# heyoeyo/muggled_dpt

Hardware: AMD Instinct MI355X
Metric: depth-maps/sec @518x518 (504x504 model tensor), Depth-Anything-V2 ViT-L (higher is better)
Workload: dtype bf16; 1 GPU; Depth-Anything-V2 ViT-L (vitl), 518x518 image -> 504x504 tensor, batch 32/GPU, bf16 MFMA operands + fp32 accumulate, mdpt_forward via C ABI; global_batch=32, parallelism=dp1, gemm_tile=0, batch_split=True

## Files before the change

### muggled_dpt_amd/csrc/gemm.hip

```cpp

#include "mdpt_kernels.h"
#include "mdpt_prof.h"
#include "f8_cross.h"
#include <stdio.h>
#include <stdlib.h>

#pragma clang fp contract(off)

typedef __attribute__((ext_vector_type(16))) float f32x16;
typedef __attribute__((ext_vector_type(4))) float f32x4;

namespace {

#include "gemm_common.inc"
#include "gemm_epilogue_strip.inc"
#include "gemm_lockstep.inc"
#include "gemm8_epilogues.inc"
#include "gemm8.inc"

template <int AMODE, int EKIND, int DMODE, bool F8 = false>
int launch_pp_mode(const GemmParams& p, hipStream_t stream) {
    constexpr unsigned LDS = 2 * 65536;
    if constexpr (MDPT_OP_IS_F16 && !F8 && (EKIND == MDPT_E_GENERIC || EKIND == MDPT_E_D2S) && DMODE != DM_RINIT) {
        if (p.f8) return launch_pp_mode<AMODE, EKIND, DMODE, true>(p, stream);
    }
    auto kern = gemm8_kernel<AMODE, EKIND, DMODE, F8>;
    static bool attr_done = false;
    if (!attr_done) {
        hipError_t e = hipFuncSetAttribute((const void*)kern, hipFuncAttributeMaxDynamicSharedMemorySize, LDS);
        if (e != hipSuccess) return (int)e;
        attr_done = true;
    }
    const int tiles = ((p.M + 255) / 256) * ((p.N + 255) / 256);
    static char prof_name[64] = "";
    if (!prof_name[0]) snprintf(prof_name, sizeof(prof_name), F8 ? "gemm8_kernel<%d, %d, %d, f8>" : "gemm8_kernel<%d, %d, %d>", AMODE, EKIND, DMODE);
    MdptProfScope prof(prof_name, 2.0 * (p.M_alg > 0 ? p.M_alg : p.M) * p.N * p.K, stream);
    const int ks = (AMODE == MDPT_A_DENSE && EKIND == MDPT_E_GENERIC && DMODE == DM_F32 && p.ksplit > 1) ? p.ksplit : 1;
    hipLaunchKernelGGL(kern, dim3(tiles, ks), dim3(512), LDS, stream, p);
    return (int)hipGetLastError();
}

template <int AMODE, int EKIND>
int launch_pp(const GemmParams& p, hipStream_t stream) {
    if constexpr (EKIND == MDPT_E_GENERIC) {
        const int dmode = generic_direct_mode(p);
// ... 134 lines not shown
```

### muggled_dpt_amd/csrc/gemm8.inc

```
template <int AMODE, bool F8 = false>
struct HalfStager {
    static constexpr int A_BYTES = 256 * 128;
#ifdef MDPT_GEMM8_BUF_STAGING
    static constexpr bool BUFFERED = AMODE != MDPT_A_CONV3;
#else
    static constexpr bool BUFFERED = false;
#endif
    __amdgpu_buffer_rsrc_t rs_a, rs_w;
    unsigned a_voff[4], b_voff;
    int a_soff, b_soff, a_row_step, b_row_step;
    const op_t* a_base_hi; const op_t* a_base_lo; const op_t* w_base_hi; const op_t* w_base_lo;
    size_t a_bytes, w_bytes;
    const op_t* a_ptr[4];
    int a_pix[4], a_y[4], a_x[4], a_ko[4];
    const op_t* b_ptr[4];
    ptrdiff_t a_hi_minus_lo, w_lo_minus_hi;
    const op_t* conv_plane;
    int a_pass, a_k0, a_tap, a_ci, b_pass, b_k0;
    int st_m0, st_n0, b_step;
    bool a_f8, b_f8;

    __device__ __forceinline__ void place_a(const GemmParams& p, int pass, int wave, int lane) {
        const int lrow = lane >> 3;
        a_f8 = pass < p.npass - 1;
// ... 188 lines not shown
        }
        }
        if (F8 && H == 1 && b_f8) {
            b_k0 += 128;
            if (b_k0 == p.K) {
                b_k0 = 0;
                ++b_pass;
                place_b(p, b_pass, wave, threadIdx.x & 63);
            }
        } else
        if (H == 1) {
            b_k0 += 64;
            if (b_k0 == p.K) {
                b_k0 = 0;
                const ptrdiff_t dw = (b_pass == 0 ? w_lo_minus_hi : -w_lo_minus_hi) - p.K;
#pragma unroll
                for (int i = 0; i < 4; ++i) b_ptr[i] += dw;
                ++b_pass;
            }
        }
    }
};

template <int AMODE, int EKIND, bool SW, bool RI = false, bool FAST = false, bool F8 = false>
__device__ __forceinline__ void gemm8_body(const GemmParams& p, char* smem, const int dmode, const int m0, const int n0,
                                           const unsigned long long t_start) {
    static_assert(!RI || SW, "residual-initialised accumulators use the swapped operand order (4 consecutive columns per lane)");
    static_assert(!F8 || (!FAST && !RI && MDPT_HAVE_F8), "fp8 cross terms: state-machine stager, fp16 build");
    static_assert(!FAST || AMODE == MDPT_A_DENSE, "the stateless staging is for dense rows");
    constexpr int A_BYTES = 256 * 128, BUF = 2 * A_BYTES;
    const int tid = threadIdx.x, lane = tid & 63;
    const int wave = __builtin_amdgcn_readfirstlane(tid >> 6);
    const int grp = wave >> 2, wc = wave & 3;
    unsigned long long t_first = 0, t_loop = 0;
    constexpr bool swapped = SW;
    HalfStager<AMODE, F8> st;
    if constexpr (!FAST) st.init(p, m0, n0, wave, lane);
    typedef __attribute__((address_space(3))) void* lds_ptr_t;
    __amdgpu_buffer_rsrc_t rs_a, rs_w;
    unsigned fa_voff = 0, fb_voff = 0;
    int fa_step = 0, fb_step = 0;
    if constexpr (FAST) {
        const int rows_here = p.M - m0 < 256 ? p.M - m0 : 256, cols_here = p.N - n0 < 256 ? p.N - n0 : 256;
        rs_a = tile_rsrc(p.A_hi + (size_t)m0 * p.lda, (size_t)rows_here * p.lda * 2);
        rs_w = tile_rsrc(p.W_hi + (size_t)n0 * p.ldw, ((size_t)(cols_here - 1) * p.ldw + p.K) * 2);
        const int r = wave * 8 + (lane >> 3);
        const int koff = ((lane & 7) ^ ((r >> 1) & 7)) * 8;
        fa_voff = (unsigned)(r * p.lda + koff) * 2u;
        fb_voff = (unsigned)(r * p.ldw + koff) * 2u;
        fa_step = 64 * p.lda * 2;
        fb_step = 64 * p.ldw * 2;
    }
#define ISSUE_A(H_, BUF_, KB_)                                                                                          \
    do {                                                                                                                \
        if constexpr (FAST) {                                                                                           \
            _Pragma("unroll") for (int i = 2 * (H_); i < 2 * (H_) + 2; ++i)                                             \
                __builtin_amdgcn_raw_ptr_buffer_load_lds(rs_a, (lds_ptr_t)((BUF_) + (wave + 8 * i) * 1024), 16, fa_voff, (KB_) + i * fa_step, 0, 0); \
        } else {                                                                                                        \
            st.template issue_a<H_>(p, BUF_, wave);                                                                     \
        }                                                                                                               \
    } while (0)
#define ISSUE_B(H_, BUF_, KB_)                                                                                          \
    do {                                                                                                                \
        if constexpr (FAST) {                                                                                           \
            _Pragma("unroll") for (int i = 2 * (H_); i < 2 * (H_) + 2; ++i)                                             \
                __builtin_amdgcn_raw_ptr_buffer_load_lds(rs_w, (lds_ptr_t)((BUF_) + 256 * 128 + (wave + 8 * i) * 1024), 16, fb_voff, (KB_) + i * fb_step, 0, 0); \
        } else {                                                                                                        \
            st.template issue_b<H_>(p, BUF_, wave);                                                                     \
        }                                                                                                               \
    } while (0)

    const int l15 = lane & 15, lh = lane >> 4, key = (l15 >> 1) & 7;
    const int a_off0 = (grp * 64 + l15) * 128 + ((lh ^ key) << 4), a_off1 = (grp * 64 + l15) * 128 + (((4 + lh) ^ key) << 4);
    const int b_off0 = A_BYTES + (wc * 32 + l15) * 128 + ((lh ^ key) << 4), b_off1 = A_BYTES + (wc * 32 + l15) * 128 + (((4 + lh) ^ key) << 4);

// ... 52 lines not shown
    do {                                                                                                              \
        if constexpr (swapped) f8_mfma16_w_first<2 * (QN_) + (J_)>(acc[QM_][QN_][I_][J_], f8_cat(FB_[J_][0], FB_[J_][1]), f8_cat(fa[I_][0], fa[I_][1]), WS_, asc); \
        else f8_mfma16_a_first<2 * (QN_) + (J_)>(acc[QM_][QN_][I_][J_], f8_cat(fa[I_][0], fa[I_][1]), f8_cat(FB_[J_][0], FB_[J_][1]), asc, WS_); \
    } while (0)
#define MFMA_Q8(QM_, QN_, FB_, WS_)                                                                                   \
    do {                                                                                                              \
        __builtin_amdgcn_s_setprio(1);                                                                                \
        MFMA_Q8_ONE(QM_, QN_, FB_, 0, 0, WS_); MFMA_Q8_ONE(QM_, QN_, FB_, 0, 1, WS_);                                 \
        MFMA_Q8_ONE(QM_, QN_, FB_, 1, 0, WS_); MFMA_Q8_ONE(QM_, QN_, FB_, 1, 1, WS_);                                 \
        MFMA_Q8_ONE(QM_, QN_, FB_, 2, 0, WS_); MFMA_Q8_ONE(QM_, QN_, FB_, 2, 1, WS_);                                 \
        MFMA_Q8_ONE(QM_, QN_, FB_, 3, 0, WS_); MFMA_Q8_ONE(QM_, QN_, FB_, 3, 1, WS_);                                 \
        __builtin_amdgcn_s_setprio(0);                                                                                \
    } while (0)
#endif
#define WAIT_LGKM(N_) asm volatile("s_waitcnt lgkmcnt(" #N_ ")" ::: "memory")
#define WAIT_VM(N_) asm volatile("s_waitcnt vmcnt(" #N_ ")" ::: "memory")
#define ACC_READY(QM_, QN_, N_)                                                                                                          \
    asm volatile("s_waitcnt vmcnt(" #N_ ")"                                                                                              \
                 : "+v"(acc[QM_][QN_][0][0]), "+v"(acc[QM_][QN_][0][1]), "+v"(acc[QM_][QN_][1][0]), "+v"(acc[QM_][QN_][1][1]),           \
                   "+v"(acc[QM_][QN_][2][0]), "+v"(acc[QM_][QN_][2][1]), "+v"(acc[QM_][QN_][3][0]), "+v"(acc[QM_][QN_][3][1])            \
                 :                                                                                                                       \
                 : "memory")

    const int T = F8 ? ktiles_total(p, p.K) : (p.K / 64) * p.npass;
    const int T8 = F8 ? ktiles_f8(p, p.K) : 0, T8a = F8 ? p.K / 128 : 0;
    char* const bufE = smem;
    char* const bufO = smem + BUF;
    ISSUE_A(0, bufE, 0);
    ISSUE_B(0, bufE, 0);
    ISSUE_B(1, bufE, 0);
    ISSUE_A(1, bufE, 0);
    if constexpr (RI) {
        constexpr unsigned OOB = 0xFFFFFFF0u;
        typedef __attribute__((ext_vector_type(4))) int i32x4;
        const int rows_here = p.M - m0 < 256 ? p.M - m0 : 256;
        const unsigned long long base = (unsigned long long)(p.resid + (size_t)m0 * p.ldr);
        i32x4 rs;
        rs[0] = __builtin_amdgcn_readfirstlane((int)(unsigned)base);
        rs[1] = __builtin_amdgcn_readfirstlane((int)(unsigned)(base >> 32) & 0xFFFF);
        rs[2] = __builtin_amdgcn_readfirstlane((int)(unsigned)((size_t)rows_here * p.ldr * 4));
        rs[3] = 0x00020000;
        const unsigned row_b = (unsigned)p.ldr * 4u;
        auto load_quadrant = [&](int qm, int qn) {
#pragma unroll
            for (int j = 0; j < 2; ++j) {
                const int nc = n0 + qn * 128 + wc * 32 + j * 16 + 4 * lh;
                const unsigned col = nc < p.N ? (unsigned)nc * 4u : OOB;
#pragma unroll
                for (int i = 0; i < 4; ++i) {
                    const unsigned row = (unsigned)(qm * 128 + grp * 64 + i * 16 + l15) * row_b;
                    const unsigned off = col == OOB ? OOB : row + col;
                    asm volatile("s_nop 4\n\tbuffer_load_dwordx4 %0, %1, %2, 0 offen" : "=v"(acc[qm][qn][i][j]) : "v"(off), "s"(rs) : "memory");
                }
            }
        };
        load_quadrant(0, 0);
        ISSUE_B(0, bufO, 128);
        ISSUE_A(0, bufO, 128);
        ISSUE_B(1, bufO, 128);
        ISSUE_A(1, bufO, 128);
        load_quadrant(0, 1);
        load_quadrant(1, 1);
        load_quadrant(1, 0);
        WAIT_VM(40);
    } else {
        ISSUE_B(0, bufO, 128);
        ISSUE_A(0, bufO, 128);
        ISSUE_B(1, bufO, 128);
        ISSUE_A(1, bufO, 128);
        WAIT_VM(8);
    }
    BAR();
    if (p.dbg_times) t_first = memtime_now();
    if (grp == 1) BAR();


    const float ri_scale = (MDPT_OP_IS_F16 && RI && p.wscale) ? p.wscale[0] : 1.0f;
#define SCALE_Q(QM_, QN_)                                                                                             \
    do {                                                                                                              \
        if (MDPT_OP_IS_F16 && RI && ri_scale != 1.0f) {                                                               \
            _Pragma("unroll") for (int i = 0; i < 4; ++i)                                                             \
                _Pragma("unroll") for (int j = 0; j < 2; ++j) acc[QM_][QN_][i][j] *= ri_scale;                        \
        }                                                                                                             \
    } while (0)
#define GEMM8_ITER(MORE_, FIRST_, MQ)                                                                                       \
    do {                                                                                                              \
        const int kE = t * 128 + 256, kO = kE + 128;         \
                                                                                                              \
        LOAD_B(fb0, 0, 0); PIN(); LOAD_A(0, 0); PIN();                                                                \
        WAIT_LGKM(8); BAR(); WAIT_LGKM(0); PIN();                                                                     \
        if (FIRST_) { ACC_READY(0, 0, 32); SCALE_Q(0, 0); PIN(); }                     \
        MQ(0, 0, fb0); BAR();                                                                                     \
                                                                                                              \
        LOAD_B(fb1, 1, 0); PIN();                                                                                     \
        if (MORE_) ISSUE_B(0, bufE, kE);                                                             \
        BAR(); WAIT_LGKM(0); PIN();                                                                                   \
        if (FIRST_) { ACC_READY(0, 1, 18); SCALE_Q(0, 1); PIN(); }                               \
        MQ(0, 1, fb1); BAR();                                                                                     \
                                                                                                              \
        LOAD_A(1, 0); PIN();                                                                                          \
        if (MORE_) ISSUE_A(0, bufE, kE);                                                             \
        PIN(); WAIT_LGKM(0); BAR(); PIN();                                                                            \
        if (FIRST_) { ACC_READY(1, 1, 12); SCALE_Q(1, 1); PIN(); }                                \
        MQ(1, 1, fb1); BAR();                                                                                     \
                                                                                                              \
        if (MORE_) { ISSUE_B(1, bufE, kE); ISSUE_A(1, bufE, kE); PIN(); WAIT_VM(8); } else { WAIT_VM(0); }                      \
        BAR();                                                                                                        \
        if (FIRST_) { ACC_READY(1, 0, 8); SCALE_Q(1, 0); PIN(); }  \
        MQ(1, 0, fb0); BAR();                                                                                     \
                                                                                                              \
        LOAD_B(fb0, 0, 1); PIN(); LOAD_A(0, 1); PIN();                                                                \
        WAIT_LGKM(8); BAR(); WAIT_LGKM(0); PIN();                                                                     \
        MQ(0, 0, fb0); BAR();                                                                                     \
                                                                                                              \
        LOAD_B(fb1, 1, 1); PIN();                                                                                     \
        if (MORE_) ISSUE_B(0, bufO, kO);                                                             \
        BAR(); WAIT_LGKM(0); PIN();                                                                                   \
        MQ(0, 1, fb1); BAR();                                                                                     \
                                                                                                              \
        LOAD_A(1, 1); PIN();                                                                                          \
        if (MORE_) ISSUE_A(0, bufO, kO);                                                             \
        PIN(); WAIT_LGKM(0); BAR(); PIN();                                                                            \
        MQ(1, 1, fb1); BAR();                                                                                     \
                                                                                                              \
        if (MORE_) { ISSUE_B(1, bufO, kO); ISSUE_A(1, bufO, kO); PIN(); WAIT_VM(8); }                                          \
        BAR();                                                                                                        \
        MQ(1, 0, fb0); BAR();                                                                                     \
    } while (0)
    if constexpr (FAST) {
        int t = 0;
        if constexpr (RI) {
            GEMM8_ITER(true, true, MFMA_Q);
            t = 2;
        }
        for (; t + 2 < T; t += 2) GEMM8_ITER(true, false, MFMA_Q);
        GEMM8_ITER(false, false, MFMA_Q);
    } else {
        int t = 0;
#if MDPT_HAVE_F8
        if constexpr (F8) {
#define MQ8A(QM_, QN_, FB_) MFMA_Q8(QM_, QN_, FB_, wsc)
#define MQ8B(QM_, QN_, FB_) MFMA_Q8(QM_, QN_, FB_, wsc_lo)
            for (; t < T8a; t += 2) GEMM8_ITER(true, false, MQ8A);
            for (; t < T8; t += 2) GEMM8_ITER(true, false, MQ8B);
#undef MQ8A
#undef MQ8B
        }
#endif
        for (; t < T; t += 2) {
            const bool more = t + 2 < T;
            GEMM8_ITER(more, (RI && t == 0), MFMA_Q);
        }
    }
#undef GEMM8_ITER
#undef SCALE_Q
#undef ACC_READY
#undef ISSUE_A
#undef ISSUE_B
    if (grp == 0) BAR();
#undef LOAD_A
#undef LOAD_B
#undef MFMA_Q
#if MDPT_HAVE_F8
#undef MFMA_Q8
#undef MFMA_Q8_ONE
#endif
    if (p.dbg_times) t_loop = memtime_now();
    if constexpr (SW) {
        if (EKIND == MDPT_E_SWQKV) {
            if (dmode == DM_F32) {
                if (HAVE_IMGB && p.bias_img_stride) epilogue_direct<DM_F32, false, MDPT_ACT_NONE, HAVE_IMGB>(p, acc, m0, n0, grp, wc, lane);
                else epilogue_direct<DM_F32, false, MDPT_ACT_NONE>(p, acc, m0, n0, grp, wc, lane);
            } else if (HAVE_IMGB && p.bias_img_stride) {
                if (p.q_lo) epilogue_swin_qk<true, HAVE_IMGB>(p, acc, m0, n0, grp, wc, lane);
// ... 16 lines not shown
            } else {
                if (p.out_lo) epilogue_direct<DM_BF16, true, MDPT_ACT_NONE, HAVE_IMGB>(p, acc, m0, n0, grp, wc, lane);
                else epilogue_direct<DM_BF16, false, MDPT_ACT_NONE, HAVE_IMGB>(p, acc, m0, n0, grp, wc, lane);
            }
        } else if (dmode == DM_BF16) {
            const int sel = (p.out_lo ? 3 : 0) + (p.act == MDPT_ACT_GELU ? 2 : (p.act == MDPT_ACT_RELU || p.relu_bf16) ? 1 : 0);
            switch (sel) {
                case 0: epilogue_direct<DM_BF16, false, MDPT_ACT_NONE>(p, acc, m0, n0, grp, wc, lane); break;
                case 1: epilogue_direct<DM_BF16, false, MDPT_ACT_RELU>(p, acc, m0, n0, grp, wc, lane); break;
                case 2: epilogue_direct<DM_BF16, false, MDPT_ACT_GELU>(p, acc, m0, n0, grp, wc, lane); break;
                case 3: epilogue_direct<DM_BF16, true, MDPT_ACT_NONE>(p, acc, m0, n0, grp, wc, lane); break;
                case 4: epilogue_direct<DM_BF16, true, MDPT_ACT_RELU>(p, acc, m0, n0, grp, wc, lane); break;
                default: epilogue_direct<DM_BF16, true, MDPT_ACT_GELU>(p, acc, m0, n0, grp, wc, lane); break;
            }
        } else if (dmode == DM_F32 || dmode == DM_RINIT) {
            if (HAVE_IMGB && p.bias_img_stride) epilogue_direct<DM_F32, false, MDPT_ACT_NONE, HAVE_IMGB>(p, acc, m0, n0, grp, wc, lane);
            else epilogue_direct<DM_F32, false, MDPT_ACT_NONE>(p, acc, m0, n0, grp, wc, lane);
        } else {
            epilogue_direct<DM_RESID, false, MDPT_ACT_NONE>(p, acc, m0, n0, grp, wc, lane);
        }
        if (p.dbg_times && tid == 0) {
            const unsigned long long t_issued = memtime_now();
            asm volatile("s_waitcnt vmcnt(0)" ::: "memory");
            unsigned long long* d = p.dbg_times + (size_t)blockIdx.x * 6;
            d[0] = t_start; d[1] = t_first; d[2] = t_loop; d[3] = memtime_now();
            d[4] = t_issued;
            d[5] = __builtin_amdgcn_s_getreg(4 << 0 | 0 << 6 | 31 << 11);
        }
        return;
    }
    if ((EKIND == MDPT_E_QKV && dmode == DM_VT) || (EKIND == MDPT_E_SWQKV && dmode == DM_SWVT)) {
        if (EKIND == MDPT_E_SWQKV) {
            if (HAVE_IMGB && p.bias_img_stride) {
                if (p.vt_lo) epilogue_swin_vt<true, HAVE_IMGB>(p, acc, m0, n0, grp, wc, lane);
                else epilogue_swin_vt<false, HAVE_IMGB>(p, acc, m0, n0, grp, wc, lane);
            } else if (p.vt_lo) epilogue_swin_vt<true>(p, acc, m0, n0, grp, wc, lane);
            else epilogue_swin_vt<false>(p, acc, m0, n0, grp, wc, lane);
        } else if (HAVE_IMGB && p.bias_img_stride) {
            if (p.vt_lo) epilogue_direct_vt<true, HAVE_IMGB>(p, acc, m0, n0, grp, wc, lane);
            else epilogue_direct_vt<false, HAVE_IMGB>(p, acc, m0, n0, grp, wc, lane);
        } else if (p.vt_lo) {
            epilogue_direct_vt<true>(p, acc, m0, n0, grp, wc, lane);
        } else {
            epilogue_direct_vt<false>(p, acc, m0, n0, grp, wc, lane);
        }
        if (p.dbg_times && tid == 0) {
            asm volatile("s_waitcnt vmcnt(0)" ::: "memory");
// ... 23 lines not shown
        asm volatile("s_waitcnt vmcnt(0)" ::: "memory");
        unsigned long long* d = p.dbg_times + (size_t)blockIdx.x * 6;
        d[0] = t_start; d[1] = t_first; d[2] = t_loop; d[3] = memtime_now();
        d[4] = __builtin_amdgcn_s_getreg(20 << 0 | 0 << 6 | 3 << 11);
        d[5] = __builtin_amdgcn_s_getreg(4 << 0 | 0 << 6 | 31 << 11);
    }
}
#undef PIN
#undef BAR
#undef WAIT_LGKM
#undef WAIT_VM

__host__ __device__ inline int generic_direct_mode(const GemmParams& p) {
    const bool imgb_ok = HAVE_IMGB && p.bias_img_rows >= 256 && p.bias && !p.gamma && !p.relu_bf16 && p.act != MDPT_ACT_RELU;
    const bool plain = !p.up_src && (!p.bias_img_stride || imgb_ok);
    const bool fits = (size_t)256 * p.ldc * 4 < 0xFFFFFFF0ull;
    if (plain && fits && p.out_hi && !p.out_f32 && !p.gamma && !p.resid && !(p.relu_bf16 && p.act != MDPT_ACT_NONE)) return DM_BF16;
    if (plain && fits && !p.bias_img_stride && p.out_f32 && !p.out_hi && p.gamma && p.resid && p.resid == p.out_f32 && p.bias && p.act == MDPT_ACT_NONE && p.ldr == p.ldc)
        return DM_RESID;
    if (plain && fits && p.acc_init && p.out_f32 && !p.out_hi && !p.gamma && p.resid == p.out_f32 && p.ldr == p.ldc && p.act == MDPT_ACT_NONE && !p.relu_bf16)
        return DM_RINIT;
    if (plain && fits && p.out_f32 && !p.out_hi && !p.gamma && !p.resid && p.act == MDPT_ACT_NONE && !p.relu_bf16) return DM_F32;
    return DM_NONE;
}

template <int AMODE, int EKIND, int DMODE, bool F8 = false>
__global__ __launch_bounds__(512, 1) void gemm8_kernel(const GemmParams p) {
    extern __shared__ __attribute__((aligned(16))) char smem[];
    unsigned long long t_start = 0;
    if (p.dbg_times) t_start = memtime_now();
    int m0, n0;
    tile_coords((p.N + 255) / 256, 256, 256, m0, n0);
    if constexpr (EKIND == MDPT_E_SWQKV) {
        const bool fast = p.npass == 1;
        if (n0 >= 2 * p.F && p.swin_vtokmap) {
            if (fast) gemm8_body<AMODE, EKIND, false, false, true>(p, smem, DM_SWVT, m0, n0, t_start);
            else gemm8_body<AMODE, EKIND, false>(p, smem, DM_SWVT, m0, n0, t_start);
        } else {
            const int dm = n0 >= 2 * p.F ? DM_F32 : DM_SWQK;
            if (fast) gemm8_body<AMODE, EKIND, true, false, true>(p, smem, dm, m0, n0, t_start);
            else gemm8_body<AMODE, EKIND, true>(p, smem, dm, m0, n0, t_start);
        }
    } else if (EKIND == MDPT_E_QKV) {
#ifdef MDPT_GEMM8_NO_FAST
        const bool fast = false;
#else
// ... 49 lines not shown
```

### muggled_dpt_amd/csrc/gemm8_epilogues.inc

```
constexpr bool HAVE_IMGB = MDPT_OP_IS_F16 != 0;
enum { DM_NONE = 0, DM_BF16 = 1, DM_RESID = 2, DM_QK = 3, DM_VT = 4, DM_F32 = 5, DM_RINIT = 6, DM_SWQK = 7, DM_SWVT = 8 };

__device__ __forceinline__ __amdgpu_buffer_rsrc_t tile_rsrc(const void* base, size_t bytes) {
    return __builtin_amdgcn_make_buffer_rsrc(const_cast<void*>(base), 0, (int)(unsigned)(bytes < 0xFFFFFFF0ull ? bytes : 0xFFFFFFF0ull), 0x00020000);
}

template <int MODE, bool X3, int ACT, bool IMGB = false>
__device__ __forceinline__ void epilogue_direct(const GemmParams& p, f32x4 (&acc)[2][2][4][2], int m0, int n0, int grp, int wc, int lane) {
    typedef __attribute__((ext_vector_type(2))) float f32x2;
    typedef __attribute__((ext_vector_type(4))) unsigned u32x4;
    constexpr unsigned OOB = 0xFFFFFFF0u;
    const int l15 = lane & 15, lh = lane >> 4;
    const int rows_here = p.M - m0 < 256 ? p.M - m0 : 256;
    int bnd = 1 << 30;
    const float* bias0 = p.bias;
    const float* bias1 = p.bias;
    if (IMGB) {
        const int img0 = m0 / p.bias_img_rows;
        bnd = (img0 + 1) * p.bias_img_rows - m0;
        bias0 = p.bias + (size_t)img0 * p.bias_img_stride;
        bias1 = bnd < rows_here ? bias0 + p.bias_img_stride : bias0;
    }
    auto pick = [&](const f32x4& a, const f32x4& b, bool next) {
        f32x4 r;
#pragma unroll
        for (int e = 0; e < 4; ++e) r[e] = next ? b[e] : a[e];
        return r;
    };

    if (MODE == DM_F32) {
        const __amdgpu_buffer_rsrc_t rs = tile_rsrc(p.out_f32 + (size_t)m0 * p.ldc, (size_t)rows_here * p.ldc * 4);
        const unsigned row_b = (unsigned)p.ldc * 4u;
        const float inv_s = (MDPT_OP_IS_F16 && p.wscale) ? p.wscale[1] : 1.0f;
#pragma unroll
        for (int qn = 0; qn < 2; ++qn) {
            f32x4 bias[2], biasn[2];
            unsigned col_off[2];
#pragma unroll
            for (int j = 0; j < 2; ++j) {
                const int nc = n0 + qn * 128 + wc * 32 + j * 16 + 4 * lh;
                bias[j] = p.bias ? *(const f32x4*)(bias0 + (nc < p.N ? nc : p.N - 4)) : f32x4{0.0f, 0.0f, 0.0f, 0.0f};
                if (IMGB) biasn[j] = *(const f32x4*)(bias1 + (nc < p.N ? nc : p.N - 4));
                col_off[j] = nc < p.N ? (unsigned)nc * 4u : OOB;
            }
#pragma unroll
            for (int qm = 0; qm < 2; ++qm)
#pragma unroll
                for (int i = 0; i < 4; ++i) {
                    const unsigned row = (unsigned)(qm * 128 + grp * 64 + i * 16 + l15) * row_b;
                    const bool next = IMGB && qm * 128 + grp * 64 + i * 16 + l15 >= bnd;
#pragma unroll
                    for (int j = 0; j < 2; ++j) {
                        const f32x4 a = MDPT_OP_IS_F16 ? acc[qm][qn][i][j] * inv_s : acc[qm][qn][i][j];
                        const f32x4 v = a + (IMGB ? pick(bias[j], biasn[j], next) : bias[j]);
                        __builtin_amdgcn_raw_buffer_store_b128(__builtin_bit_cast(u32x4, v), rs, col_off[j] == OOB ? OOB : row + col_off[j], 0, 0);
                    }
                }
        }
        return;
    }
    if (MODE == DM_RESID) {
        const __amdgpu_buffer_rsrc_t rs = tile_rsrc(p.out_f32 + (size_t)m0 * p.ldc, (size_t)rows_here * p.ldc * 4);
        const unsigned row_b = (unsigned)p.ldc * 4u;
        f32x4 bias[2][2], gam[2][2];
        unsigned col_off[2][2];
#pragma unroll
        for (int qn = 0; qn < 2; ++qn)
#pragma unroll
            for (int j = 0; j < 2; ++j) {
                const int nc = n0 + qn * 128 + wc * 32 + j * 16 + 4 * lh;
                const int ncl = nc < p.N ? nc : p.N - 4;
                bias[qn][j] = *(const f32x4*)(p.bias + ncl);
                gam[qn][j] = *(const f32x4*)(p.gamma + ncl);
                col_off[qn][j] = nc < p.N ? (unsigned)nc * 4u : OOB;
            }
        auto row_off = [&](int g, int i) { return (unsigned)((g >> 1) * 128 + grp * 64 + i * 16 + l15) * row_b; };
        u32x4 old[4][4][2];
        f32x4 res[2][4][2];
        auto load_group = [&](int g) {
#pragma unroll
// ... 454 lines not shown
```

### muggled_dpt_amd/csrc/gemm_common.inc

```
__device__ __forceinline__ void glds16(const void* gsrc, char* lds_wave_base) {
    __builtin_amdgcn_global_load_lds((const __attribute__((address_space(1))) void*)gsrc,
                                     (__attribute__((address_space(3))) void*)lds_wave_base, 16, 0, 0);
}

__device__ __forceinline__ unsigned long long memtime_now() {
    unsigned long long t;
    asm volatile("s_memtime %0\n\ts_waitcnt lgkmcnt(0)" : "=s"(t)::"memory");
    return t;
}

#define MDPT_GELU_Q0 1.1511051654815674f
#define MDPT_GELU_Q1 0.4592081904411316f
#define MDPT_GELU_Q2 0.052496179938316345f
#define MDPT_GELU_Q3 -0.00706342002376914f
#define MDPT_GELU_Q4 0.00013693643268197775f
#define MDPT_GELU_Q5 0.00018618021567817777f
#define MDPT_GELU_Q6 -3.93776863347739e-05f
#define MDPT_GELU_Q7 2.8349124931992264e-06f
__device__ __forceinline__ float gelu_erf(float v) {
    const float a = fabsf(v);
    float q = MDPT_GELU_Q7;
    q = __builtin_fmaf(q, a, MDPT_GELU_Q6);
    q = __builtin_fmaf(q, a, MDPT_GELU_Q5);
    q = __builtin_fmaf(q, a, MDPT_GELU_Q4);
// ... 172 lines not shown
        st_k0 += BK;
        if (AMODE == MDPT_A_CONV3) {
            st_sub += BK;
            if (st_sub == 64) {
                st_sub = 0;
                if (++st_tap == 9) { st_tap = 0; st_ci += 64; }
            }
        }
        if (st_k0 == kspan) {
            st_k0 = 0; st_tap = st_tap0; st_ci = st_ci0; st_sub = 0;
            const ptrdiff_t da = (st_pass == 0 ? a_hi_minus_lo : 0) - kspan;
            const ptrdiff_t dw = (st_pass == 0 ? w_lo_minus_hi : -w_lo_minus_hi) - kspan;
            if (st_pass == 0) conv_plane = p.A_hi;
#pragma unroll
            for (int i = 0; i < CA; ++i)
                if (AMODE != MDPT_A_CONV3) a_ptr[i] += da;
#pragma unroll
            for (int i = 0; i < CB; ++i) b_ptr[i] += dw;
            ++st_pass;
        }
    }
};

__device__ __forceinline__ void tile_coords(int tiles_n, int BM, int BN, int& m0, int& n0) {
    const int nwg = gridDim.x, bid = blockIdx.x;
    const int xq = nwg >> 3, xr = nwg & 7, xcd = bid & 7;
    const int swz = (xcd < xr ? xcd * (xq + 1) : xr * (xq + 1) + (xcd - xr) * xq) + (bid >> 3);
    if (tiles_n >= 8 && (tiles_n & 3) == 0) {
        const int tiles_m = nwg / tiles_n, per_panel = tiles_m * 4;
        const int panel = swz / per_panel, r = swz - panel * per_panel;
        m0 = (r >> 2) * BM;
        n0 = (panel * 4 + (r & 3)) * BN;
        return;
    }
    m0 = (swz / tiles_n) * BM;
    n0 = (swz % tiles_n) * BN;
}
```

### muggled_dpt_amd/csrc/mdpt_debug.cpp

```cpp
#include "mdpt_internal.h"

extern "C" {

int mdpt_debug_set_stop(mdpt_handle* h, int32_t block, int32_t step) {
    if (!h) return fail(MDPT_E_INVALID, "null handle");
    h->dbg_block = block; h->dbg_step = step;
    return 0;
}

int mdpt_debug_set_reassemble_overlap(mdpt_handle* h, int32_t on) {
    if (!h) return fail(MDPT_E_INVALID, "null handle");
    if (on < 0 || on > 2) return fail(MDPT_E_INVALID, "reassemble overlap: 0 = off, 1 = the library's rule, 2 = always");
    h->overlap_reasm = on;
    return 0;
}

int mdpt_debug_set_wscale_policy(mdpt_handle* h, int32_t all) {
    if (!h) return fail(MDPT_E_INVALID, "null handle");
    h->wscale_all = all ? 1 : 0;
    h->finalized = false;
    return 0;
}

int mdpt_debug_set_side_stream_priority(mdpt_handle* h, int32_t prio) {
// ... 85 lines not shown
    return 0;
}

int mdpt_debug_gemm(const void* a_bf16, const void* w_bf16, void* out_f32, void* out_bf16, int32_t M, int32_t N, int32_t K,
                    int32_t tile, int32_t iters, void* stream, void* dbg_times) {
    if (!a_bf16 || !w_bf16 || (!out_f32 && !out_bf16)) return fail(MDPT_E_INVALID, "null argument");
    GemmParams g;
    memset(&g, 0, sizeof(g));
    g.A_hi = (const op_t*)a_bf16; g.W_hi = (const op_t*)w_bf16;
    g.M = M; g.N = N; g.K = K; g.lda = K; g.npass = 1;
    g.zero_page = (const op_t*)w_bf16;
    g.amode = MDPT_A_DENSE; g.ekind = MDPT_E_GENERIC; g.tile = tile & 255;
    g.act = (tile >> 8) & 3;
    g.out_f32 = (float*)out_f32; g.out_hi = (op_t*)out_bf16; g.ldc = N; g.ldr = N;
    g.dbg_times = (unsigned long long*)dbg_times;
    if ((tile >> 10) & 1) {
        if (!out_f32 || !out_bf16) return fail(MDPT_E_INVALID, "residual mode needs both output buffers");
        g.bias = (const float*)out_bf16; g.gamma = (const float*)out_bf16 + N; g.resid = (const float*)out_f32; g.out_hi = nullptr;
    }
    if ((tile >> 11) & 1) {
        if (!out_f32 || !out_bf16) return fail(MDPT_E_INVALID, "residual mode needs both output buffers");
        g.bias = (const float*)out_bf16; g.resid = (const float*)out_f32; g.out_hi = nullptr; g.acc_init = 1;
    }
    for (int i = 0; i < iters; ++i) CHK(OPLG(mdpt_launch_gemm, g, (hipStream_t)stream));
    return 0;
}

int mdpt_debug_conv3(const void* in_bf16, const void* w_packed_bf16, const void* bias_f32, const void* skip_f32, const void* up_f32, int32_t Hu,
                     int32_t Wu, void* out_f32, void* out_bf16, int32_t relu_bf16, int32_t B, int32_t H, int32_t W, int32_t Cin, int32_t Cout,
                     int32_t path, int32_t tile, int32_t iters, void* stream, void* dbg_times, const void* in_lo_bf16, const void* w_lo_bf16,
                     void* out_lo_bf16) {
    if (Cout != 256 && Cout != 128) return fail(MDPT_E_INVALID, "Cout must be 256 or 128");
    if (w_lo_bf16 && !in_lo_bf16) return fail(MDPT_E_INVALID, "a lo plane of the weights needs one of the input (three passes); the input alone = two passes");
    if (!in_bf16 || !w_packed_bf16 || (!out_bf16 && !out_f32)) return fail(MDPT_E_INVALID, "null argument");
    static op_t* zero_page = nullptr;
    if (!zero_page) {
        if (hipMalloc((void**)&zero_page, 256) != hipSuccess || hipMemset(zero_page, 0, 256) != hipSuccess) return fail(MDPT_E_STATE, "zero page allocation failed");
    }
    if (path == 2 || path == 3) {
        if (Cout != 128 || !out_bf16 || Hu < 2 || Wu < 2) return fail(MDPT_E_INVALID, "upsampled-input form: 128 output channels, bf16 output");
        if (path == 2) {
            Conv3hParams q;
            memset(&q, 0, sizeof(q));
            q.up_in = (const op_t*)in_bf16; q.Hs = Hu; q.Ws = Wu; q.w = (const op_t*)w_packed_bf16; q.bias = (const float*)bias_f32;
            q.out_bf = (op_t*)out_bf16; q.B = B; q.H = H; q.W = W; q.Cin = Cin; q.Cout = 128;
            q.dbg_times = (unsigned long long*)dbg_times;
// ... 75 lines not shown
```

### muggled_dpt_amd/csrc/mdpt_kernels.h

```cpp
#pragma once
#include <hip/hip_runtime.h>
#include <stddef.h>
#include <stdint.h>

#include "op_types.h"

enum { MDPT_DT_F32 = 0, MDPT_DT_BF16 = 1, MDPT_DT_F16 = 2 };

enum { MDPT_A_DENSE = 0, MDPT_A_TOKENS = 1, MDPT_A_CONV3 = 2 };
enum { MDPT_E_GENERIC = 0, MDPT_E_QKV = 1, MDPT_E_PATCH = 2, MDPT_E_D2S = 3, MDPT_E_HEAD = 4, MDPT_E_SWQKV = 5 };
enum { MDPT_ACT_NONE = 0, MDPT_ACT_RELU = 1, MDPT_ACT_GELU = 2 };
enum { MDPT_TILE_AUTO = 0, MDPT_TILE_128x128 = 1, MDPT_TILE_256x256 = 2, MDPT_TILE_128x32 = 3, MDPT_TILE_256x128 = 4, MDPT_TILE_PP256 = 5, MDPT_TILE_64x64 = 6 };

struct GemmParams {
    const op_t* A_hi; const op_t* A_lo;
    const op_t* W_hi; const op_t* W_lo;
    int M, N, K;
    int ldw;
    int M_alg;
    int lda;
    int npass;
    const op_t* zero_page;
    int amode, ekind, tile;
    int tok_np, tok_stride;
// ... 1 lines not shown
    const float* bias; const float* gamma; const float* resid; int ldr;
    int bias_img_stride, bias_img_rows;
    const float* up_src; int Hu, Wu;
    int act;
    float* out_f32; op_t* out_hi; op_t* out_lo; int ldc;
    int relu_bf16;
    int acc_init;
    const float* wscale;
    op_t* q_hi; op_t* q_lo; op_t* k_hi; op_t* k_lo; op_t* vt_hi; op_t* vt_lo;
    int F, heads, npad, npadv; float qscale;
    const int* swin_tokmap; const float* swin_logit_scale; int swin_N, swin_img_rows;
    const int* swin_vtokmap; int swin_img_velems;
    const float* pos;
    int d2s_k, d2s_cout;
    const float* head_w; const float* head_b; int head_sigmoid; void* head_out; int head_out_dtype;
    int throughput_mode;
    int f8; size_t a8_off;
    const unsigned char* W8; const unsigned char* W8_lo;
    const unsigned char* S8; const unsigned char* S8_lo;
    size_t out_f8; int out_a8;
    int ksplit; float* ks_part;
    int ks_all;
    unsigned long long* dbg_times;
};


struct Conv3hParams {
    const op_t* in;
    const op_t* up_in; int Hs, Ws;
    const op_t* in_lo;
    const op_t* w;
    const op_t* w_lo;
    const float* bias;
    const float* skip;
    const float* up_src; int Hu, Wu;
    float* out_f32;
    op_t* out_bf;
    op_t* out_bf_lo;
    int relu_bf;
    int B, H, W, Cin;
    int Cout;
    int f8; size_t a8_off;
    const unsigned char* w8; const unsigned char* w8_lo; const unsigned char* s8; const unsigned char* s8_lo;
    size_t out_f8; int out_a8;
    unsigned long long* dbg_times;
};
// ... 114 lines not shown
```

Baseline: 768.8 depth-maps/s.

## Add persistent tile-walking kernel for residual-initialised dense GEMM

Adds a persistent variant of the residual-initialised (DM_RINIT) dense GEMM. One workgroup per CU loops over output tiles. It prefetches the next tile's operands while finishing the current one, and overlaps the previous tile's fp32 epilogue stores with the residual loads that initialise the next tile's accumulators. The aim is to hide per-tile prologue and epilogue latency and to remove wave-quantisation tails when tiles outnumber CUs. The cost is more complex control flow, register pressure, and new ACC_READY wait counts that must match the changed load ordering.

```diff
diff --git a/muggled_dpt_amd/csrc/gemm.hip b/muggled_dpt_amd/csrc/gemm.hip
--- a/muggled_dpt_amd/csrc/gemm.hip
+++ b/muggled_dpt_amd/csrc/gemm.hip
@@ -18,9 +18,44 @@
 #include "gemm8_epilogues.inc"
 #include "gemm8.inc"
 
+int rinit_persistent_grid(const GemmParams& p, int tiles) {
+    if (p.npass != 1 || (p.N & 255) || p.bias_img_stride || p.wscale || p.rinit_grid < 0) return 0;
+    if (p.rinit_grid > 0) return p.rinit_grid < tiles ? p.rinit_grid : tiles;
+#ifdef MDPT_DEBUG_SWITCHES
+    static const bool off = getenv("MDPT_GEMM_NO_PERSIST") != nullptr;
+    if (off) return 0;
+#endif
+    static int cus = 0;
+    if (!cus) {
+        int dev = 0, n = 0;
+        if (hipGetDevice(&dev) != hipSuccess || hipDeviceGetAttribute(&n, hipDeviceAttributeMultiprocessorCount, dev) != hipSuccess || n < 8) return 0;
+        cus = n & ~7;
+    }
+    return tiles >= 2 * cus ? cus : 0;
+}
+
+int launch_rinit_persistent(const GemmParams& p_in, int grid, hipStream_t stream) {
+    constexpr unsigned LDS = 2 * 65536;
+    static bool attr_done = false;
+    if (!attr_done) {
+        hipError_t e = hipFuncSetAttribute((const void*)gemm8_rinit_persistent_kernel, hipFuncAttributeMaxDynamicSharedMemorySize, LDS);
+        if (e != hipSuccess) return (int)e;
+        attr_done = true;
+    }
+    GemmParams p = p_in;
+    p.ptiles = ((p.M + 255) / 256) * ((p.N + 255) / 256);
+    MdptProfScope prof("gemm8_kernel<0, 0, 6, persistent>", 2.0 * (p.M_alg > 0 ? p.M_alg : p.M) * p.N * p.K, stream);
+    hipLaunchKernelGGL(gemm8_rinit_persistent_kernel, dim3(grid), dim3(512), LDS, stream, p);
+    return (int)hipGetLastError();
+}
+
 template <int AMODE, int EKIND, int DMODE, bool F8 = false>
 int launch_pp_mode(const GemmParams& p, hipStream_t stream) {
     constexpr unsigned LDS = 2 * 65536;
+    if constexpr (AMODE == MDPT_A_DENSE && EKIND == MDPT_E_GENERIC && DMODE == DM_RINIT && !F8) {
+        const int grid = rinit_persistent_grid(p, ((p.M + 255) / 256) * ((p.N + 255) / 256));
+        if (grid > 0) return launch_rinit_persistent(p, grid, stream);
+    }
     if constexpr (MDPT_OP_IS_F16 && !F8 && (EKIND == MDPT_E_GENERIC || EKIND == MDPT_E_D2S) && DMODE != DM_RINIT) {
         if (p.f8) return launch_pp_mode<AMODE, EKIND, DMODE, true>(p, stream);
     }
diff --git a/muggled_dpt_amd/csrc/gemm8.inc b/muggled_dpt_amd/csrc/gemm8.inc
--- a/muggled_dpt_amd/csrc/gemm8.inc
+++ b/muggled_dpt_amd/csrc/gemm8.inc
@@ -234,10 +234,11 @@
     }
 };
 
-template <int AMODE, int EKIND, bool SW, bool RI = false, bool FAST = false, bool F8 = false>
-__device__ __forceinline__ void gemm8_body(const GemmParams& p, char* smem, const int dmode, const int m0, const int n0,
-                                           const unsigned long long t_start) {
+template <int AMODE, int EKIND, bool SW, bool RI = false, bool FAST = false, bool F8 = false, bool PERSIST = false>
+__device__ __forceinline__ void gemm8_body(const GemmParams& p, char* smem, const int dmode, int m0, int n0,
+                                           unsigned long long t_start) {
     static_assert(!RI || SW, "residual-initialised accumulators use the swapped operand order (4 consecutive columns per lane)");
+    static_assert(!PERSIST || (RI && FAST), "the tile walk exists for the residual-initialised form with stateless staging");
     static_assert(!F8 || (!FAST && !RI && MDPT_HAVE_F8), "fp8 cross terms: state-machine stager, fp16 build");
     static_assert(!FAST || AMODE == MDPT_A_DENSE, "the stateless staging is for dense rows");
     constexpr int A_BYTES = 256 * 128, BUF = 2 * A_BYTES;
@@ -245,6 +246,7 @@
     const int wave = __builtin_amdgcn_readfirstlane(tid >> 6);
     const int grp = wave >> 2, wc = wave & 3;
     unsigned long long t_first = 0, t_loop = 0;
+    int vb = (int)blockIdx.x;
     constexpr bool swapped = SW;
     HalfStager<AMODE, F8> st;
     if constexpr (!FAST) st.init(p, m0, n0, wave, lane);
@@ -263,6 +265,11 @@
         fa_step = 64 * p.lda * 2;
         fb_step = 64 * p.ldw * 2;
     }
+    auto place_operands = [&](int tm0, int tn0) {
+        const int rows_here = p.M - tm0 < 256 ? p.M - tm0 : 256, cols_here = p.N - tn0 < 256 ? p.N - tn0 : 256;
+        rs_a = tile_rsrc(p.A_hi + (size_t)tm0 * p.lda, (size_t)rows_here * p.lda * 2);
+        rs_w = tile_rsrc(p.W_hi + (size_t)tn0 * p.ldw, ((size_t)(cols_here - 1) * p.ldw + p.K) * 2);
+    };
 #define ISSUE_A(H_, BUF_, KB_)                                                                                          \
     do {                                                                                                                \
         if constexpr (FAST) {                                                                                           \
@@ -361,6 +368,32 @@
                  :                                                                                                                       \
                  : "memory")
 
+    typedef __attribute__((ext_vector_type(4))) int i32x4;
+    i32x4 rs_r = {0, 0, 0, 0};
+    int r_n0 = n0;
+    auto resid_rsrc = [&](int tm0) {
+        const int rows_here = p.M - tm0 < 256 ? p.M - tm0 : 256;
+        const unsigned long long base = (unsigned long long)(p.resid + (size_t)tm0 * p.ldr);
+        rs_r[0] = __builtin_amdgcn_readfirstlane((int)(unsigned)base);
+        rs_r[1] = __builtin_amdgcn_readfirstlane((int)(unsigned)(base >> 32) & 0xFFFF);
+        rs_r[2] = __builtin_amdgcn_readfirstlane((int)(unsigned)((size_t)rows_here * p.ldr * 4));
+        rs_r[3] = 0x00020000;
+    };
+    auto load_quadrant = [&](int qm, int qn, int l15, int lh) {
+        constexpr unsigned OOB = 0xFFFFFFF0u;
+        const unsigned row_b = (unsigned)p.ldr * 4u;
+#pragma unroll
+        for (int j = 0; j < 2; ++j) {
+            const int nc = r_n0 + qn * 128 + wc * 32 + j * 16 + 4 * lh;
+            const unsigned col = nc < p.N ? (unsigned)nc * 4u : OOB;
+#pragma unroll
+            for (int i = 0; i < 4; ++i) {
+                const unsigned row = (unsigned)(qm * 128 + grp * 64 + i * 16 + l15) * row_b;
+                const unsigned off = col == OOB ? OOB : row + col;
+                asm volatile("s_nop 4\n\tbuffer_load_dwordx4 %0, %1, %2, 0 offen" : "=v"(acc[qm][qn][i][j]) : "v"(off), "s"(rs_r) : "memory");
+            }
+        }
+    };
     const int T = F8 ? ktiles_total(p, p.K) : (p.K / 64) * p.npass;
     const int T8 = F8 ? ktiles_f8(p, p.K) : 0, T8a = F8 ? p.K / 128 : 0;
     char* const bufE = smem;
@@ -369,38 +402,23 @@
     ISSUE_B(0, bufE, 0);
     ISSUE_B(1, bufE, 0);
     ISSUE_A(1, bufE, 0);
-    if constexpr (RI) {
-        constexpr unsigned OOB = 0xFFFFFFF0u;
-        typedef __attribute__((ext_vector_type(4))) int i32x4;
-        const int rows_here = p.M - m0 < 256 ? p.M - m0 : 256;
-        const unsigned long long base = (unsigned long long)(p.resid + (size_t)m0 * p.ldr);
-        i32x4 rs;
-        rs[0] = __builtin_amdgcn_readfirstlane((int)(unsigned)base);
-        rs[1] = __builtin_amdgcn_readfirstlane((int)(unsigned)(base >> 32) & 0xFFFF);
-        rs[2] = __builtin_amdgcn_readfirstlane((int)(unsigned)((size_t)rows_here * p.ldr * 4));
-        rs[3] = 0x00020000;
-        const unsigned row_b = (unsigned)p.ldr * 4u;
-        auto load_quadrant = [&](int qm, int qn) {
-#pragma unroll
-            for (int j = 0; j < 2; ++j) {
-                const int nc = n0 + qn * 128 + wc * 32 + j * 16 + 4 * lh;
-                const unsigned col = nc < p.N ? (unsigned)nc * 4u : OOB;
-#pragma unroll
-                for (int i = 0; i < 4; ++i) {
-                    const unsigned row = (unsigned)(qm * 128 + grp * 64 + i * 16 + l15) * row_b;
-                    const unsigned off = col == OOB ? OOB : row + col;
-                    asm volatile("s_nop 4\n\tbuffer_load_dwordx4 %0, %1, %2, 0 offen" : "=v"(acc[qm][qn][i][j]) : "v"(off), "s"(rs) : "memory");
-                }
-            }
-        };
-        load_quadrant(0, 0);
+    if constexpr (PERSIST) {
         ISSUE_B(0, bufO, 128);
         ISSUE_A(0, bufO, 128);
         ISSUE_B(1, bufO, 128);
         ISSUE_A(1, bufO, 128);
-        load_quadrant(0, 1);
-        load_quadrant(1, 1);
-        load_quadrant(1, 0);
+    } else
+    if constexpr (RI) {
+        resid_rsrc(m0);
+        r_n0 = n0;
+        load_quadrant(0, 0, l15, lh);
+        ISSUE_B(0, bufO, 128);
+        ISSUE_A(0, bufO, 128);
+        ISSUE_B(1, bufO, 128);
+        ISSUE_A(1, bufO, 128);
+        load_quadrant(0, 1, l15, lh);
+        load_quadrant(1, 1, l15, lh);
+        load_quadrant(1, 0, l15, lh);
         WAIT_VM(40);
     } else {
         ISSUE_B(0, bufO, 128);
@@ -409,10 +427,11 @@
         ISSUE_A(1, bufO, 128);
         WAIT_VM(8);
     }
-    BAR();
-    if (p.dbg_times) t_first = memtime_now();
-    if (grp == 1) BAR();
-
+    if constexpr (!PERSIST) {
+        BAR();
+        if (p.dbg_times) t_first = memtime_now();
+        if (grp == 1) BAR();
+    }
 
     const float ri_scale = (MDPT_OP_IS_F16 && RI && p.wscale) ? p.wscale[0] : 1.0f;
 #define SCALE_Q(QM_, QN_)                                                                                             \
@@ -422,25 +441,25 @@
                 _Pragma("unroll") for (int j = 0; j < 2; ++j) acc[QM_][QN_][i][j] *= ri_scale;                        \
         }                                                                                                             \
     } while (0)
-#define GEMM8_ITER(MORE_, FIRST_, MQ)                                                                                       \
+#define GEMM8_ITER(MORE_, FIRST_, MQ, R1_, R2_, R3_)                                                                                     \
     do {                                                                                                              \
         const int kE = t * 128 + 256, kO = kE + 128;         \
                                                                                                               \
         LOAD_B(fb0, 0, 0); PIN(); LOAD_A(0, 0); PIN();                                                                \
         WAIT_LGKM(8); BAR(); WAIT_LGKM(0); PIN();                                                                     \
-        if (FIRST_) { ACC_READY(0, 0, 32); SCALE_Q(0, 0); PIN(); }                     \
+        if (FIRST_) { ACC_READY(0, 0, R1_); SCALE_Q(0, 0); PIN(); }                  \
         MQ(0, 0, fb0); BAR();                                                                                     \
                                                                                                               \
         LOAD_B(fb1, 1, 0); PIN();                                                                                     \
         if (MORE_) ISSUE_B(0, bufE, kE);                                                             \
         BAR(); WAIT_LGKM(0); PIN();                                                                                   \
-        if (FIRST_) { ACC_READY(0, 1, 18); SCALE_Q(0, 1); PIN(); }                               \
+        if (FIRST_) { ACC_READY(0, 1, R2_); SCALE_Q(0, 1); PIN(); }                             \
         MQ(0, 1, fb1); BAR();                                                                                     \
                                                                                                               \
         LOAD_A(1, 0); PIN();                                                                                          \
         if (MORE_) ISSUE_A(0, bufE, kE);                                                             \
         PIN(); WAIT_LGKM(0); BAR(); PIN();                                                                            \
-        if (FIRST_) { ACC_READY(1, 1, 12); SCALE_Q(1, 1); PIN(); }                                \
+        if (FIRST_) { ACC_READY(1, 1, R3_); SCALE_Q(1, 1); PIN(); }                             \
         MQ(1, 1, fb1); BAR();                                                                                     \
                                                                                                               \
         if (MORE_) { ISSUE_B(1, bufE, kE); ISSUE_A(1, bufE, kE); PIN(); WAIT_VM(8); } else { WAIT_VM(0); }                      \
@@ -468,27 +487,85 @@
     } while (0)
     if constexpr (FAST) {
         int t = 0;
+        if constexpr (PERSIST) {
+            const int tiles_n = (p.N + 255) / 256;
+#pragma unroll
+            for (int a = 0; a < 2; ++a)
+#pragma unroll
+                for (int b = 0; b < 2; ++b)
+#pragma unroll
+                    for (int i = 0; i < 4; ++i)
+#pragma unroll
+                        for (int j = 0; j < 2; ++j) acc[a][b][i][j] = f32x4{0.0f, 0.0f, 0.0f, 0.0f};
+            __amdgpu_buffer_rsrc_t rs_o = tile_rsrc(p.out_f32, 0);
+            int pn0 = n0, pvb = -1;
+            for (;;) {
+                {
+                    int lane_o = lane;
+                    asm volatile("" : "+v"(lane_o));
+                    const int l15 = lane_o & 15, lh = lane_o >> 4;
+                    const unsigned row_b = (unsigned)p.ldc * 4u;
+                    const float inv_s = (MDPT_OP_IS_F16 && p.wscale) ? p.wscale[1] : 1.0f;
+                    F32Cols c0, c1;
+                    epilogue_f32_cols<false>(p, p.bias, p.bias, pn0, 0, wc, lh, c0);
+                    epilogue_f32_cols<false>(p, p.bias, p.bias, pn0, 1, wc, lh, c1);
+                    asm volatile("s_waitcnt vmcnt(0)" : "+v"(c0.bias[0]), "+v"(c0.bias[1]), "+v"(c1.bias[0]), "+v"(c1.bias[1]) : : "memory");
+                    resid_rsrc(m0);
+                    r_n0 = n0;
+                    PIN();
+                    epilogue_f32_store<false>(c0, acc, rs_o, row_b, inv_s, 0, 0, grp, l15, 1 << 30); PIN(); load_quadrant(0, 0, l15, lh); PIN();
+                    epilogue_f32_store<false>(c1, acc, rs_o, row_b, inv_s, 0, 1, grp, l15, 1 << 30); PIN(); load_quadrant(0, 1, l15, lh); PIN();
+                    epilogue_f32_store<false>(c1, acc, rs_o, row_b, inv_s, 1, 1, grp, l15, 1 << 30); PIN(); load_quadrant(1, 1, l15, lh); PIN();
+                    epilogue_f32_store<false>(c0, acc, rs_o, row_b, inv_s, 1, 0, grp, l15, 1 << 30); PIN(); load_quadrant(1, 0, l15, lh); PIN();
+                }
+                if (p.dbg_times && tid == 0 && pvb >= 0) {
+                    unsigned long long* d = p.dbg_times + (size_t)pvb * 6;
+                    d[0] = t_start; d[1] = t_first; d[2] = t_loop; d[3] = d[4] = t_start = memtime_now();
+                    d[5] = __builtin_amdgcn_s_getreg(4 << 0 | 0 << 6 | 31 << 11);
+                }
+                BAR();
+                if (p.dbg_times) t_first = memtime_now();
+                if (grp == 1) BAR();
+                t = 0;
+                GEMM8_ITER(true, true, MFMA_Q, 48, 34, 20);
+                for (t = 2; t + 2 < T; t += 2) GEMM8_ITER(true, false, MFMA_Q, 0, 0, 0);
+                const int vnext = vb + (int)gridDim.x;
+                if (vnext >= p.ptiles) break;
+                int nm0, nn0;
+                tile_coords_of(p.ptiles, vnext, tiles_n, 256, 256, nm0, nn0);
+                place_operands(nm0, nn0);
+                t = -2;
+                GEMM8_ITER(true, false, MFMA_Q, 0, 0, 0);
+                if (grp == 0) BAR();
+                if (p.dbg_times) t_loop = memtime_now();
+                rs_o = tile_rsrc(p.out_f32 + (size_t)m0 * p.ldc, (size_t)(p.M - m0 < 256 ? p.M - m0 : 256) * p.ldc * 4);
+                pn0 = n0; pvb = vb;
+                m0 = nm0; n0 = nn0; vb = vnext;
+            }
+            GEMM8_ITER(false, false, MFMA_Q, 0, 0, 0);
+        } else {
         if constexpr (RI) {
-            GEMM8_ITER(true, true, MFMA_Q);
+            GEMM8_ITER(true, true, MFMA_Q, 32, 18, 12);
             t = 2;
         }
-        for (; t + 2 < T; t += 2) GEMM8_ITER(true, false, MFMA_Q);
-        GEMM8_ITER(false, false, MFMA_Q);
+        for (; t + 2 < T; t += 2) GEMM8_ITER(true, false, MFMA_Q, 0, 0, 0);
+        GEMM8_ITER(false, false, MFMA_Q, 0, 0, 0);
+        }
     } else {
         int t = 0;
 #if MDPT_HAVE_F8
         if constexpr (F8) {
 #define MQ8A(QM_, QN_, FB_) MFMA_Q8(QM_, QN_, FB_, wsc)
 #define MQ8B(QM_, QN_, FB_) MFMA_Q8(QM_, QN_, FB_, wsc_lo)
-            for (; t < T8a; t += 2) GEMM8_ITER(true, false, MQ8A);
-            for (; t < T8; t += 2) GEMM8_ITER(true, false, MQ8B);
+            for (; t < T8a; t += 2) GEMM8_ITER(true, false, MQ8A, 0, 0, 0);
+            for (; t < T8; t += 2) GEMM8_ITER(true, false, MQ8B, 0, 0, 0);
 #undef MQ8A
 #undef MQ8B
         }
 #endif
         for (; t < T; t += 2) {
             const bool more = t + 2 < T;
-            GEMM8_ITER(more, (RI && t == 0), MFMA_Q);
+            GEMM8_ITER(more, (RI && t == 0), MFMA_Q, 32, 18, 12);
         }
     }
 #undef GEMM8_ITER
@@ -551,7 +628,7 @@
         if (p.dbg_times && tid == 0) {
             const unsigned long long t_issued = memtime_now();
             asm volatile("s_waitcnt vmcnt(0)" ::: "memory");
-            unsigned long long* d = p.dbg_times + (size_t)blockIdx.x * 6;
+            unsigned long long* d = p.dbg_times + (size_t)vb * 6;
             d[0] = t_start; d[1] = t_first; d[2] = t_loop; d[3] = memtime_now();
             d[4] = t_issued;
             d[5] = __builtin_amdgcn_s_getreg(4 << 0 | 0 << 6 | 31 << 11);
@@ -621,6 +698,15 @@
         return DM_RINIT;
     if (plain && fits && p.out_f32 && !p.out_hi && !p.gamma && !p.resid && p.act == MDPT_ACT_NONE && !p.relu_bf16) return DM_F32;
     return DM_NONE;
+}
+
+__global__ __launch_bounds__(512, 1) void gemm8_rinit_persistent_kernel(const GemmParams p) {
+    extern __shared__ __attribute__((aligned(16))) char smem[];
+    unsigned long long t_start = 0;
+    if (p.dbg_times) t_start = memtime_now();
+    int m0, n0;
+    tile_coords_of(p.ptiles, (int)blockIdx.x, (p.N + 255) / 256, 256, 256, m0, n0);
+    gemm8_body<MDPT_A_DENSE, MDPT_E_GENERIC, true, true, true, false, true>(p, smem, DM_RINIT, m0, n0, t_start);
 }
 
 template <int AMODE, int EKIND, int DMODE, bool F8 = false>
diff --git a/muggled_dpt_amd/csrc/gemm8_epilogues.inc b/muggled_dpt_amd/csrc/gemm8_epilogues.inc
--- a/muggled_dpt_amd/csrc/gemm8_epilogues.inc
+++ b/muggled_dpt_amd/csrc/gemm8_epilogues.inc
@@ -3,6 +3,40 @@
 
 __device__ __forceinline__ __amdgpu_buffer_rsrc_t tile_rsrc(const void* base, size_t bytes) {
     return __builtin_amdgcn_make_buffer_rsrc(const_cast<void*>(base), 0, (int)(unsigned)(bytes < 0xFFFFFFF0ull ? bytes : 0xFFFFFFF0ull), 0x00020000);
+}
+
+struct F32Cols { f32x4 bias[2], biasn[2]; unsigned col_off[2]; };
+template <bool IMGB>
+__device__ __forceinline__ void epilogue_f32_cols(const GemmParams& p, const float* bias0, const float* bias1, int n0, int qn, int wc, int lh, F32Cols& c) {
+#pragma unroll
+    for (int j = 0; j < 2; ++j) {
+        const int nc = n0 + qn * 128 + wc * 32 + j * 16 + 4 * lh;
+        c.bias[j] = p.bias ? *(const f32x4*)(bias0 + (nc < p.N ? nc : p.N - 4)) : f32x4{0.0f, 0.0f, 0.0f, 0.0f};
+        if (IMGB) c.biasn[j] = *(const f32x4*)(bias1 + (nc < p.N ? nc : p.N - 4));
+        c.col_off[j] = nc < p.N ? (unsigned)nc * 4u : 0xFFFFFFF0u;
+    }
+}
+template <bool IMGB>
+__device__ __forceinline__ void epilogue_f32_store(const F32Cols& c, const f32x4 (&acc)[2][2][4][2], const __amdgpu_buffer_rsrc_t rs, unsigned row_b, float inv_s,
+                                                   int qm, int qn, int grp, int l15, int bnd) {
+    typedef __attribute__((ext_vector_type(4))) unsigned u32x4;
+    constexpr unsigned OOB = 0xFFFFFFF0u;
+#pragma unroll
+    for (int i = 0; i < 4; ++i) {
+        const unsigned row = (unsigned)(qm * 128 + grp * 64 + i * 16 + l15) * row_b;
+        const bool next = IMGB && qm * 128 + grp * 64 + i * 16 + l15 >= bnd;
+#pragma unroll
+        for (int j = 0; j < 2; ++j) {
+            const f32x4 a = MDPT_OP_IS_F16 ? acc[qm][qn][i][j] * inv_s : acc[qm][qn][i][j];
+            f32x4 b = c.bias[j];
+            if (IMGB) {
+#pragma unroll
+                for (int e = 0; e < 4; ++e) b[e] = next ? c.biasn[j][e] : c.bias[j][e];
+            }
+            const f32x4 v = a + b;
+            __builtin_amdgcn_raw_buffer_store_b128(__builtin_bit_cast(u32x4, v), rs, c.col_off[j] == OOB ? OOB : row + c.col_off[j], 0, 0);
+        }
+    }
 }
 
 template <int MODE, bool X3, int ACT, bool IMGB = false>
@@ -34,28 +68,10 @@
         const float inv_s = (MDPT_OP_IS_F16 && p.wscale) ? p.wscale[1] : 1.0f;
 #pragma unroll
         for (int qn = 0; qn < 2; ++qn) {
-            f32x4 bias[2], biasn[2];
-            unsigned col_off[2];
-#pragma unroll
-            for (int j = 0; j < 2; ++j) {
-                const int nc = n0 + qn * 128 + wc * 32 + j * 16 + 4 * lh;
-                bias[j] = p.bias ? *(const f32x4*)(bias0 + (nc < p.N ? nc : p.N - 4)) : f32x4{0.0f, 0.0f, 0.0f, 0.0f};
-                if (IMGB) biasn[j] = *(const f32x4*)(bias1 + (nc < p.N ? nc : p.N - 4));
-                col_off[j] = nc < p.N ? (unsigned)nc * 4u : OOB;
-            }
-#pragma unroll
-            for (int qm = 0; qm < 2; ++qm)
-#pragma unroll
-                for (int i = 0; i < 4; ++i) {
-                    const unsigned row = (unsigned)(qm * 128 + grp * 64 + i * 16 + l15) * row_b;
-                    const bool next = IMGB && qm * 128 + grp * 64 + i * 16 + l15 >= bnd;
-#pragma unroll
-                    for (int j = 0; j < 2; ++j) {
-                        const f32x4 a = MDPT_OP_IS_F16 ? acc[qm][qn][i][j] * inv_s : acc[qm][qn][i][j];
-                        const f32x4 v = a + (IMGB ? pick(bias[j], biasn[j], next) : bias[j]);
-                        __builtin_amdgcn_raw_buffer_store_b128(__builtin_bit_cast(u32x4, v), rs, col_off[j] == OOB ? OOB : row + col_off[j], 0, 0);
-                    }
-                }
+            F32Cols c;
+            epilogue_f32_cols<IMGB>(p, bias0, bias1, n0, qn, wc, lh, c);
+#pragma unroll
+            for (int qm = 0; qm < 2; ++qm) epilogue_f32_store<IMGB>(c, acc, rs, row_b, inv_s, qm, qn, grp, l15, bnd);
         }
         return;
     }
diff --git a/muggled_dpt_amd/csrc/gemm_common.inc b/muggled_dpt_amd/csrc/gemm_common.inc
--- a/muggled_dpt_amd/csrc/gemm_common.inc
+++ b/muggled_dpt_amd/csrc/gemm_common.inc
@@ -218,8 +218,7 @@
     }
 };
 
-__device__ __forceinline__ void tile_coords(int tiles_n, int BM, int BN, int& m0, int& n0) {
-    const int nwg = gridDim.x, bid = blockIdx.x;
+__device__ __forceinline__ void tile_coords_of(int nwg, int bid, int tiles_n, int BM, int BN, int& m0, int& n0) {
     const int xq = nwg >> 3, xr = nwg & 7, xcd = bid & 7;
     const int swz = (xcd < xr ? xcd * (xq + 1) : xr * (xq + 1) + (xcd - xr) * xq) + (bid >> 3);
     if (tiles_n >= 8 && (tiles_n & 3) == 0) {
@@ -232,3 +231,6 @@
     m0 = (swz / tiles_n) * BM;
     n0 = (swz % tiles_n) * BN;
 }
+__device__ __forceinline__ void tile_coords(int tiles_n, int BM, int BN, int& m0, int& n0) {
+    tile_coords_of((int)gridDim.x, (int)blockIdx.x, tiles_n, BM, BN, m0, n0);
+}
diff --git a/muggled_dpt_amd/csrc/mdpt_debug.cpp b/muggled_dpt_amd/csrc/mdpt_debug.cpp
--- a/muggled_dpt_amd/csrc/mdpt_debug.cpp
+++ b/muggled_dpt_amd/csrc/mdpt_debug.cpp
@@ -131,6 +131,8 @@
         if (!out_f32 || !out_bf16) return fail(MDPT_E_INVALID, "residual mode needs both output buffers");
         g.bias = (const float*)out_bf16; g.resid = (const float*)out_f32; g.out_hi = nullptr; g.acc_init = 1;
     }
+    if ((tile >> 12) & 1) g.rinit_grid = -1;
+    else if ((tile >> 16) & 0x7FFF) g.rinit_grid = (tile >> 16) & 0x7FFF;
     for (int i = 0; i < iters; ++i) CHK(OPLG(mdpt_launch_gemm, g, (hipStream_t)stream));
     return 0;
 }
diff --git a/muggled_dpt_amd/csrc/mdpt_kernels.h b/muggled_dpt_amd/csrc/mdpt_kernels.h
--- a/muggled_dpt_amd/csrc/mdpt_kernels.h
+++ b/muggled_dpt_amd/csrc/mdpt_kernels.h
@@ -47,6 +47,8 @@
     int ksplit; float* ks_part;
     int ks_all;
     unsigned long long* dbg_times;
+    int rinit_grid;
+    int ptiles;
 };
 
 
```

After: 769.4 depth-maps/s (median of 2 runs). About the same (+0.1%).
